# Big-Brother-Pikachu/Where2edit

Hardware: AMD Instinct MI355X
Metric: 1024^2 edited images/sec per mapper step (higher is better)
Workload: dtype f32; 1 GPU; BASELINE configs[1]: FFHQ-1024 StyleGAN2 + clip_loss mapper step (coach.py:79-92), 4 latents/GPU, LevelsMapper, Ranger, id_lambda=0; global_batch=4, per_gpu_batch=4, micro_batch=4, parallelism=dp1, conv_precision=f32, stabilise_steps=12, stabilised=True, hip_graph=True, side_stream=False, clip_precision=f32

## Files before the change

include/w2e.h:

```cpp
#ifndef W2E_H
#define W2E_H

#include <stddef.h>
#include <stdint.h>

#ifdef __cplusplus
extern "C" {
#endif

#define W2E_VERSION 7

int w2e_version(void);
const char* w2e_last_error(void);

int w2e_set_option(const char* name, const char* value);

#define W2E_PLANAR_PITCH(w) ((((w) + 1) + 15) & ~15)
int w2e_get_option(const char* name, int* value);

int w2e_upfirdn2d(const float* x, const float* kern, float* y, int64_t planes, int in_h, int in_w, int out_h,
                  int out_w, int kh, int kw, int up, int down, int pad_x0, int pad_y0, int flip, int in_layout, int in_pitch,
                  int act, const float* out_scale, const float* noise, const float* noise_w, const float* bias,
                  int channels, float slope, float gain, void* stream);
int w2e_blur_adjoint_actbwd(const float* gy, const float* y_fwd, const float* noise, const float* kern, float* gt, float* sums,
                            int64_t planes, int h, int w, float slope, float gain, void* stream);

int w2e_bias_act_fwd(const float* x, const float* bias, const float* noise, const float* noise_w, float* y,
                     int64_t outer, int64_t channels, int64_t inner, float slope, float gain, void* stream);
int w2e_bias_act_bwd(const float* gy, const float* y, float* gx, int64_t n, float slope, float gain, void* stream);
int w2e_bias_act_bwd_reduce(const float* gy, const float* y, const float* noise, float* gx, float* sums,
                            int64_t outer, int64_t channels, int64_t inner, float slope, float gain, void* stream);

int w2e_conv_pack(const float* weight, float* wp, int cout, int cin, float scale, int transpose, int flip,
                  void* stream);

#define W2E_CONV_SAME 0
#define W2E_CONV_UP 1
#define W2E_CONV_DOWN 2

int w2e_modconv3x3(int mode, const float* x, const float* wp, const float* in_scale, const float* out_scale,
                   float* y, int batch, int k_ch, int n_ch, int h, int w, int y_pitch, int act, const float* noise,
                   const float* noise_w, const float* bias, const float* dot_with, float* dot_out, void* stream);

int w2e_wino_weights_fused(const float* wp, float* uf, int k_ch, int n_ch, void* stream);
int w2e_wino_fused(const float* x, const float* in_scale, const float* uf, const float* out_scale, float* y, int batch, int k_ch,
                   int n_ch, int h, int w, int act, const float* noise, const float* noise_w, const float* bias, const float* slope,
                   const float* dot_with, float* dot_out, int wgs, void* stream);

int w2e_wino_gemm_plan(int batch, int k_ch, int n_ch, int h, int w, int* tiles_padded, int* splits, int64_t* workspace_floats);
int w2e_wino_pack_input(const float* x, const float* in_scale, float* vf, int batch, int k_ch, int h, int w, int tiles_padded, void* stream);
int w2e_wino_gemm(const float* uf, const float* vf, const float* out_scale, float* y, int batch, int k_ch, int n_ch, int h, int w,
                  int tiles_padded, int splits, float* workspace, int act, const float* noise, const float* noise_w, const float* bias,
                  const float* slope, const float* dot_with, float* dot_out, void* stream);

int w2e_demod_fwd(const float* s, const float* wsq, float* d, int batch, int cin, int cout, float eps, void* stream);
#define W2E_DEMOD_MAX_LAYERS 32
typedef struct {
    const float* s;
    const float* wsq;
    float* d;
    int cin, cout;
} w2e_demod_layer;
int w2e_demod_all_fwd(const w2e_demod_layer* layers, int n_layers, int batch, float eps, void* stream);
int w2e_demod_bwd(const float* sums, const float* dz, const float* noise_w, const float* bias, const float* d,
                  const float* s, const float* wsq, float* gs, float* gd, int batch, int cin, int cout, void* stream);
// ... 74 lines not shown
```

where2edit_amd/_lib.py:

```python
import ctypes
import os

import torch

from . import build as _build

_P = ctypes.c_void_p
_I = ctypes.c_int
_L = ctypes.c_int64
_F = ctypes.c_float

class DemodLayer(ctypes.Structure):
    _fields_ = [("s", ctypes.c_void_p), ("wsq", ctypes.c_void_p), ("d", ctypes.c_void_p), ("cin", ctypes.c_int), ("cout", ctypes.c_int)]


_PROTOS = {
    "w2e_version": (_I, []),
    "w2e_last_error": (ctypes.c_char_p, []),
    "w2e_set_option": (_I, [ctypes.c_char_p, ctypes.c_char_p]),
    "w2e_get_option": (_I, [ctypes.c_char_p, ctypes.POINTER(ctypes.c_int)]),
    "w2e_upfirdn2d": (_I, [_P, _P, _P, _L, _I, _I, _I, _I, _I, _I, _I, _I, _I, _I, _I, _I, _I, _I, _P, _P, _P, _P, _I, _F, _F, _P]),
    "w2e_blur_adjoint_actbwd": (_I, [_P, _P, _P, _P, _P, _P, _L, _I, _I, _F, _F, _P]),
    "w2e_mapper_pixelnorm": (_I, [_P, _P, _I, _I, _I, _P, _P, _P]),
    "w2e_mapper_linear": (_I, [_I, _P, _P, _P, _P, _P, _I, _I, _I, _P, _P, _F, _F, _I, _P]),
    "w2e_mapper_wgrad": (_I, [_P, _P, _P, _P, _P, _I, _I, _I, _P, _P, _F, _F, _I, _P]),
    "w2e_mapper_gather": (_I, [_P, _P, _I, _I, _I, _P, _P, _P]),
    "w2e_mapper_transpose": (_I, [_P, _I, _P, _P]),
    "w2e_ssmapper_pixelnorm": (_I, [_P, _P, _I, _I, _P, _P]),
    "w2e_ssmapper_gather": (_I, [_P, _P, _I, _I, _P, _P]),
    "w2e_ssmapper_linear": (_I, [_I, _P, _P, _P, _P, _P, _I, _I, _P, _P, _F, _P]),
    "w2e_ssmapper_wgrad": (_I, [_P, _P, _P, _P, _P, _I, _I, _P, _P, _F, _P]),
    "w2e_bias_act_fwd": (_I, [_P, _P, _P, _P, _P, _L, _L, _L, _F, _F, _P]),
    "w2e_bias_act_bwd": (_I, [_P, _P, _P, _L, _F, _F, _P]),
    "w2e_bias_act_bwd_reduce": (_I, [_P, _P, _P, _P, _P, _L, _L, _L, _F, _F, _P]),
    "w2e_conv_pack": (_I, [_P, _P, _I, _I, _F, _I, _I, _P]),
    "w2e_modconv3x3": (_I, [_I, _P, _P, _P, _P, _P, _I, _I, _I, _I, _I, _I, _I, _P, _P, _P, _P, _P, _P]),
    "w2e_wino_weights_fused": (_I, [_P, _P, _I, _I, _P]),
    "w2e_wino_fused": (_I, [_P, _P, _P, _P, _P, _I, _I, _I, _I, _I, _I, _P, _P, _P, _P, _P, _P, _I, _P]),
    "w2e_wino_gemm_plan": (_I, [_I, _I, _I, _I, _I, ctypes.POINTER(ctypes.c_int), ctypes.POINTER(ctypes.c_int), ctypes.POINTER(ctypes.c_int64)]),
    "w2e_wino_pack_input": (_I, [_P, _P, _P, _I, _I, _I, _I, _I, _P]),
    "w2e_wino_gemm": (_I, [_P, _P, _P, _P, _I, _I, _I, _I, _I, _I, _I, _P, _I, _P, _P, _P, _P, _P, _P, _P]),
    "w2e_demod_fwd": (_I, [_P, _P, _P, _I, _I, _I, _F, _P]),
    "w2e_demod_all_fwd": (_I, [ctypes.POINTER(DemodLayer), _I, _I, _F, _P]),
    "w2e_demod_bwd": (_I, [_P, _P, _P, _P, _P, _P, _P, _P, _P, _I, _I, _I, _P]),
    "w2e_modconv_wgrad_plan": (_I, [_I, _I, _I, _I, _I, _I, ctypes.POINTER(ctypes.c_int)]),
    "w2e_modconv_wgrad": (_I, [_I, _P, _P, _P, _P, _P, _I, _I, _I, _I, _I, _I, _P]),
    "w2e_modconv_wgrad_finish": (_I, [_P, _I, _P, _P, _P, _P, _P, _P, _P, _P, _I, _I, _I, _I, _F, _P]),
    "w2e_modconv_wsq": (_I, [_P, _P, _I, _I, _I, _F, _P]),
    "w2e_fromrgb_fwd": (_I, [_P, _P, _P, _P, _I, _I, _L, _F, _P]),
    "w2e_fromrgb_bwd_rows": (_I, [_I, _L]),
    "w2e_fromrgb_bwd": (_I, [_P, _P, _P, _P, _P, _P, _P, _P, _I, _I, _L, _F, _P]),
    "w2e_mbstd_fwd": (_I, [_P, _P, _I, _I, _I, _P]),
    "w2e_mbstd_bwd": (_I, [_P, _P, _P, _I, _I, _I, _P]),
    "w2e_fromrgb_jvp": (_I, [_P, _P, _P, _P, _I, _I, _L, _F, _P]),
    "w2e_mbstd_jvp": (_I, [_P, _P, _P, _I, _I, _I, _P]),
    "w2e_mbstd_hvp": (_I, [_P, _P, _P, _P, _I, _I, _I, _P]),
    "w2e_sumsq_rows_parts": (_I, [_L]),
    "w2e_sumsq_rows": (_I, [_P, _P, _P, _I, _L, _P]),
    "w2e_style_affine_fwd": (_I, [_P, _P, _P, _P, _P, _I, _I, _I, _I, _P]),
# ... 105 lines not shown
```

where2edit_amd/csrc/common.h:

```cpp
#pragma once
#include <hip/hip_runtime.h>
#include <stdarg.h>
#include <stdint.h>
#include <stdio.h>

#include "../../include/w2e.h"

namespace w2e {

void set_error(const char* fmt, ...);

struct Options {
    int conv_precision;
    int deterministic;
    int tune_cfg, tune_cfg_splits, tune_cfg_mode;
    int tune_upall, tune_dma, tune_fuse;
    int tune_mw;
    int tune_xcd;
    int tune_print, tune_blur, tune_gemm_s;
    int tune_skip, tune_clock;
};
const Options& options();

static inline bool big_lds_once(const void* fn, unsigned* done_mask) {
    int dev = 0;
    if (hipGetDevice(&dev) != hipSuccess || dev < 0 || dev >= 32) return false;
    if (*done_mask & (1u << dev)) return true;
    if (hipFuncSetAttribute(fn, hipFuncAttributeMaxDynamicSharedMemorySize, 160 * 1024) != hipSuccess) return false;
    *done_mask |= 1u << dev;
    return true;
}

int cu_count();

#define W2E_REQUIRE(cond, ...)        \
    do {                              \
        if (!(cond)) {                \
            w2e::set_error(__VA_ARGS__); \
            return 1;                 \
// ... 25 lines not shown
```

where2edit_amd/csrc/modconv.hip:

```cpp
#include <math.h>
#include <stdlib.h>
#include <string.h>

#include <type_traits>

#include "common.h"
#include "../../include/w2e_irse.h"

namespace w2e {

typedef float f32x16 __attribute__((ext_vector_type(16)));

struct ConvParams {
    const float* x;
    const float* wp;
    const float* in_scale;
    const float* out_scale;
    float* y;
    const float* noise;
    const float* noise_w;
    const float* bias;
    const float* dot_with;
    float* dot_out;
    int batch, K, N;
    int H, W;
    int in_h, in_w;
    int out_h, out_w;
    int th, tw, tw_log2;
    int tiles_x, tiles_y, tiles_n;
    int ph, pw, plane;
    unsigned pw_magic;
    int border_wgs, groups_row, groups_col;
    int tune_skip;
    const float* slope;
    int in_off;
    int splits, k_per;
    unsigned long long* stamps;
};

enum { EPI_PLAIN = 0, EPI_ACT = 1, EPI_DOT = 2, EPI_PRELU = 3 };

constexpr int CONV_UPALL = 3;
#ifdef W2E_TUNING
#define W2E_SKIP(p, bit) ((p).tune_skip & (bit))
#else
#define W2E_SKIP(p, bit) false
#endif
#ifdef W2E_STAMPS
constexpr int STAMP_STRIDE = 8;
#else
constexpr int STAMP_STRIDE = 4;
#endif
__host__ __device__ constexpr bool is_up(int mode) { return mode == W2E_CONV_UP || mode == CONV_UPALL; }

__host__ __device__ constexpr int max_patch_slots(int mode, int tm, int nt) {
    return mode == W2E_CONV_DOWN ? (nt == 512 ? (tm >= 1024 ? 9 : 5) : (tm >= 512 ? 9 : (tm >= 256 ? 5 : (tm >= 128 ? 3 : (tm >= 64 ? 2 : 1)))))
                                 : (nt == 512 ? (tm >= 2048 ? 5 : (tm >= 1024 ? 3 : 2)) : (tm >= 512 ? 3 : (tm >= 256 ? 2 : 1)));
}

template <int MODE, int PY, int PX>
// ... 221 lines not shown
    const bool even_ok = is_row ? v <= p.W : v < p.H, odd_ok = is_row ? v < p.W : v < p.H;
    const int e_idx = is_row ? (0 * hp + p.H) * wpp + v : (0 * hp + v) * wpp + p.W;
    const int o_idx = is_row ? (1 * hp + p.H) * wpp + v : (2 * hp + v) * wpp + p.W;
    constexpr int RPW = 32 / NW;
#pragma unroll
    for (int q = 0; q < RPW; ++q) {
        const int rr = wave * RPW + q;
        const int r = rr & 15;
        float sum = 0.f;
#pragma unroll
        for (int w = 0; w < NW; ++w) sum += red[w][rr][lane];
        const int och = ob * 32 + (r & 3) + 8 * (r >> 2) + 4 * half;
        if (och >= p.N) continue;
        const float os = p.out_scale ? p.out_scale[(int64_t)b * p.N + och] : 1.f;
        float* yp = p.y + ((int64_t)b * p.N + och) * 4 * hp * wpp;
        if (rr < 16) {
            if (even_ok) yp[e_idx] = sum * os;
        } else if (odd_ok) {
            yp[o_idx] = sum * os;
        }
    }
}

template <int MODE, int EPI, int NOB, int NPB, int WO, int WP, int KC, int DMA>
__global__ __launch_bounds__(64 * WO * WP, 2) void modconv_kernel(ConvParams p) {
    constexpr int NT = 64 * WO * WP;
    constexpr int TN = 32 * NOB * WO;
    constexpr int NPX = (MODE == CONV_UPALL) ? NPB / 4 : NPB;
    constexpr int MAXX = max_patch_slots(MODE == CONV_UPALL ? W2E_CONV_UP : MODE, 32 * NPX * WP, NT);
    extern __shared__ __attribute__((aligned(16))) float smem[];
    constexpr int WS_FLOATS = (MODE == W2E_CONV_UP ? 32 : KC * 9) * TN;
    float4* ws = reinterpret_cast<float4*>(smem);
    float4* xs = reinterpret_cast<float4*>(smem + WS_FLOATS);

    const int tid = threadIdx.x, lane = tid & 63;
    const int wave = __builtin_amdgcn_readfirstlane(tid >> 6);
    const int half = lane >> 5, j = lane & 31;
    const int wo = wave / WP, wpx = wave % WP;

    int bid = blockIdx.x;
    if (is_up(MODE)) {
        if (bid < p.border_wgs) {
            if (W2E_SKIP(p, 32)) return;
            upconv_border<NT>(p, smem, bid);
            return;
        }
        bid -= p.border_wgs;
    }
    const int per_phase = (gridDim.x - p.border_wgs) >> 2;
    const int phase = (MODE == W2E_CONV_UP) ? bid / per_phase : 0;
    if (MODE == W2E_CONV_UP) bid -= phase * per_phase;
    const int ks = bid % p.splits;
    bid /= p.splits;
    const int k_lo = ks * p.k_per;
    const int k_hi = W2E_SKIP(p, 2) ? k_lo : ((k_lo + p.k_per < p.K) ? k_lo + p.k_per : p.K);
#ifdef W2E_TUNING
    if (p.stamps && tid == 0) {
        p.stamps[STAMP_STRIDE * (int64_t)blockIdx.x + 0] = __builtin_amdgcn_s_memtime();
        p.stamps[STAMP_STRIDE * (int64_t)blockIdx.x + 1] = __builtin_amdgcn_s_memrealtime();
    }
#endif
    const int tx = bid % p.tiles_x;
    bid /= p.tiles_x;
    const int ty = bid % p.tiles_y;
    bid /= p.tiles_y;
    const int b = bid % p.batch;
    const int nt = bid / p.batch;
    const int n0 = nt * TN;
    const int r0 = ty * p.th, c0 = tx * p.tw;

    int base[NPB];
#pragma unroll
    for (int pb = 0; pb < NPX; ++pb) {
        const int m = (wpx * NPX + pb) * 32 + j;
        const int ly = m >> p.tw_log2, lx = m & (p.tw - 1);
        const bool ok = ly < p.th && r0 + ly < p.H && c0 + lx < p.W;
        int off;
        if (MODE == W2E_CONV_SAME) off = ly * p.pw + lx;
        else if (is_up(MODE)) off = (ly + 1) * p.pw + lx + 1;
        else off = 2 * ly * p.pw + 2 * lx;
        if (!ok) off = is_up(MODE) ? p.pw + 1 : 0;
        base[pb] = half * p.plane + off;
    }

    f32x16 acc[NOB][NPB];
#pragma unroll
    for (int ob = 0; ob < NOB; ++ob)
#pragma unroll
        for (int pb = 0; pb < NPB; ++pb)
#pragma unroll
            for (int r = 0; r < 16; ++r) acc[ob][pb][r] = 0.f;

    const int64_t in_plane = (int64_t)p.in_h * p.in_w;
    const int patch = p.ph * p.pw;
    const int oy0 = (MODE == W2E_CONV_DOWN) ? 2 * r0 + p.in_off : r0 - 1;
    const int ox0 = (MODE == W2E_CONV_DOWN) ? 2 * c0 + p.in_off : c0 - 1;

    auto k_loop = [&](auto py_c, auto px_c) __attribute__((always_inline)) {
        constexpr int PY = decltype(py_c)::value, PX = decltype(px_c)::value;
// ... 310 lines not shown
            p.stamps[STAMP_STRIDE * (int64_t)blockIdx.x + 4] = st_wait;
            p.stamps[STAMP_STRIDE * (int64_t)blockIdx.x + 5] = st_bar;
            p.stamps[STAMP_STRIDE * (int64_t)blockIdx.x + 6] = __builtin_amdgcn_s_memtime() - st_t0;
            p.stamps[STAMP_STRIDE * (int64_t)blockIdx.x + 7] = st_issue;
        }
#endif
    };
    using I0 = std::integral_constant<int, 0>;
    using I1 = std::integral_constant<int, 1>;
    if constexpr (DMA) {
        static_assert(MODE != W2E_CONV_UP, "the per-phase UP form keeps the register pipeline");
        dma_loop(0);
    } else if (MODE == W2E_CONV_UP) {
        switch (phase) {
            case 0: k_loop(I0{}, I0{}); break;
            case 1: k_loop(I0{}, I1{}); break;
            case 2: k_loop(I1{}, I0{}); break;
            default: k_loop(I1{}, I1{}); break;
        }
    } else {
        k_loop(I0{}, I0{});
    }

    const float nw = (EPI == EPI_ACT && p.noise) ? p.noise_w[0] * 1.4142135623730951f : 0.f;
    float* red = smem;
    if (EPI == EPI_DOT) {
        __syncthreads();
        if (tid < TN) red[tid] = 0.f;
        __syncthreads();
    }
    int gy[NPB], gx[NPB];
    bool valid[NPB];
#pragma unroll
    for (int pb = 0; pb < NPB; ++pb) {
        const int m = (wpx * NPX + pb % NPX) * 32 + j;
        const int ly = m >> p.tw_log2, lx = m & (p.tw - 1);
        gy[pb] = r0 + ly;
        gx[pb] = c0 + lx;
        valid[pb] = ly < p.th && gy[pb] < p.H && gx[pb] < p.W;
    }
    int pix[NPB];
    float nz[NPB];
#pragma unroll
    for (int pb = 0; pb < NPB; ++pb) {
        const int ph_pb = (MODE == CONV_UPALL) ? pb / NPX : phase;
        if (is_up(MODE)) pix[pb] = (ph_pb * (p.H + 1) + gy[pb]) * W2E_PLANAR_PITCH(p.W) + gx[pb];
// ... 109 lines not shown
                                 int transpose, int flip) {
    const int Kd = transpose ? cout : cin, Nd = transpose ? cin : cout;
    const int64_t total = (int64_t)((Kd + 7) / 8) * 9 * 2 * Nd * 4;
    for (int64_t e = (int64_t)blockIdx.x * blockDim.x + threadIdx.x; e < total; e += (int64_t)gridDim.x * blockDim.x) {
        const int c = (int)(e & 3);
        const int n = (int)((e >> 2) % Nd);
        const int hh = (int)((e / (4 * (int64_t)Nd)) & 1);
        const int tap = (int)((e / (8 * (int64_t)Nd)) % 9);
        const int kc = (int)(e / (72 * (int64_t)Nd));
        const int k = kc * 8 + 2 * c + hh;
        float v = 0.f;
        if (k < Kd) {
            const int o = transpose ? k : n, i = transpose ? n : k;
            v = scale * w[((int64_t)o * cin + i) * 9 + (flip ? 8 - tap : tap)];
        }
        wp[e] = v;
    }
}

struct TileCfg {
    int nob, npb, wo, wp;
};

template <int MODE, int EPI, int NOB, int NPB, int WO, int WP, int KC, int DMA = 0>
static void launch_cfg(const ConvParams& p, int grid, size_t lds, hipStream_t s) {
    if (lds > 64 * 1024) {
        static unsigned done = 0;
        big_lds_once((const void*)modconv_kernel<MODE, EPI, NOB, NPB, WO, WP, KC, DMA>, &done);
    }
    modconv_kernel<MODE, EPI, NOB, NPB, WO, WP, KC, DMA><<<grid, 64 * WO * WP, lds, s>>>(p);
}

static bool dma_has_cfg(bool all_phase, int cfg) {
    return all_phase ? (cfg == 0 || cfg == 1 || cfg == 2 || cfg == 8 || cfg == 11)
                     : (cfg == 0 || cfg == 1 || cfg == 2 || cfg == 8 || cfg == 9 || cfg == 10);
}

template <int EPI>
static bool launch_x3_down(int cfg, const ConvParams& p, int grid, size_t lds, hipStream_t s) {
    if (cfg != 9) return false;
    launch_cfg<W2E_CONV_DOWN, EPI, 2, 2, 2, 4, 8, 2>(p, grid, lds, s);
    return true;
}

static bool launch_x3_up(int cfg, const ConvParams& p, int grid, size_t lds, hipStream_t s) {
    switch (cfg) {
        case 0: launch_cfg<CONV_UPALL, EPI_PLAIN, 2, 4, 2, 4, 8, 2>(p, grid, lds, s); return true;
        case 1: launch_cfg<CONV_UPALL, EPI_PLAIN, 2, 4, 1, 8, 8, 2>(p, grid, lds, s); return true;
        case 2: launch_cfg<CONV_UPALL, EPI_PLAIN, 1, 4, 1, 8, 8, 2>(p, grid, lds, s); return true;
        case 11: launch_cfg<CONV_UPALL, EPI_PLAIN, 1, 8, 1, 8, 8, 2>(p, grid, lds, s); return true;
    }
    return false;
}
// ... 397 lines not shown
#define W2E_CHECK_UP_PITCH(name)                                                                                                       \
    W2E_REQUIRE(mode != W2E_CONV_UP || y_pitch == W2E_PLANAR_PITCH(w),                                                                 \
                name ": UP output with a row pitch of %d floats, this library's layout has %d (W2E_PLANAR_PITCH, ABI %d): rebuild the caller", \
                y_pitch, W2E_PLANAR_PITCH(w), W2E_VERSION)

extern "C" int w2e_modconv3x3(int mode, const float* x, const float* wp, const float* in_scale, const float* out_scale,
                              float* y, int batch, int k_ch, int n_ch, int h, int w, int y_pitch, int act, const float* noise,
                              const float* noise_w, const float* bias, const float* dot_with, float* dot_out,
                              void* stream) {
    W2E_CHECK_UP_PITCH("modconv3x3");
    return conv_impl(mode, x, wp, in_scale, out_scale, y, batch, k_ch, n_ch, h, w, act, noise, noise_w, bias, dot_with, dot_out,
                     nullptr, 0, 0, stream);
}

extern "C" int w2e_conv3x3(int mode, const float* x, const float* wp, const float* in_scale, const float* out_scale, float* y,
                           int batch, int k_ch, int n_ch, int h, int w, int y_pitch, int down_pad, const float* bias, const float* slope,
                           void* stream) {
    W2E_CHECK_UP_PITCH("conv3x3");
    const int prelu = (bias || slope) ? 1 : 0;
    W2E_REQUIRE(!(prelu && mode == W2E_CONV_UP), "conv3x3: no bias / PReLU epilogue in UP mode");
    return conv_impl(mode, x, wp, in_scale, out_scale, y, batch, k_ch, n_ch, h, w, 0, nullptr, nullptr, bias, nullptr, nullptr,
                     slope, prelu, down_pad, stream);
}
```

where2edit_amd/csrc/runtime.hip:

```cpp
#include <stdlib.h>
#include <string.h>

#include "common.h"

namespace w2e {

static thread_local char g_err[512] = "";

void set_error(const char* fmt, ...) {
    va_list ap;
    va_start(ap, fmt);
    vsnprintf(g_err, sizeof(g_err), fmt, ap);
    va_end(ap);
}

static Options g_opt;

static int parse_precision(const char* v) { return (v && strcmp(v, "bf16x3") == 0) ? 1 : 0; }

static bool apply(Options& o, const char* name, const char* value) {
    const int iv = value ? atoi(value) : 0;
    if (!strcmp(name, "conv_precision")) o.conv_precision = parse_precision(value);
    else if (!strcmp(name, "deterministic")) o.deterministic = iv != 0;
    else if (!strcmp(name, "tune_cfg")) {
        o.tune_cfg = -1, o.tune_cfg_splits = 1, o.tune_cfg_mode = -1;
        if (value && *value) sscanf(value, "%d,%d,%d", &o.tune_cfg, &o.tune_cfg_splits, &o.tune_cfg_mode);
    } else if (!strcmp(name, "tune_upall")) o.tune_upall = (value && *value) ? iv : -1;
    else if (!strcmp(name, "tune_dma")) o.tune_dma = (value && *value) ? iv : -1;
    else if (!strcmp(name, "tune_print")) o.tune_print = iv;
    else if (!strcmp(name, "tune_blur")) o.tune_blur = iv;
    else if (!strcmp(name, "tune_gemm_s")) o.tune_gemm_s = iv;
    else if (!strcmp(name, "tune_fuse")) o.tune_fuse = (value && *value) ? iv : -1;
    else if (!strcmp(name, "tune_xcd")) o.tune_xcd = (value && *value) ? iv : -1;
    else if (!strcmp(name, "tune_mw")) o.tune_mw = (value && *value) ? iv : -1;
#ifdef W2E_TUNING
    else if (!strcmp(name, "tune_skip")) o.tune_skip = iv;
    else if (!strcmp(name, "tune_clock")) o.tune_clock = iv;
#endif
    else return false;
    return true;
}

static Options from_env() {
    Options o{};
    o.tune_cfg = -1, o.tune_cfg_splits = 1, o.tune_cfg_mode = -1, o.tune_upall = -1, o.tune_dma = -1, o.tune_fuse = -1, o.tune_xcd = -1, o.tune_mw = -1;
    static const char* const kEnv[][2] = {
        {"W2E_CONV_PRECISION", "conv_precision"}, {"W2E_DETERMINISTIC", "deterministic"}, {"W2E_TUNE_CFG", "tune_cfg"},
        {"W2E_TUNE_UPALL", "tune_upall"},         {"W2E_TUNE_DMA", "tune_dma"},           {"W2E_TUNE_PRINT", "tune_print"},
        {"W2E_TUNE_BLUR", "tune_blur"},           {"W2E_TUNE_GEMM_S", "tune_gemm_s"},     {"W2E_TUNE_FUSE", "tune_fuse"},
        {"W2E_TUNE_SKIP", "tune_skip"},           {"W2E_TUNE_CLOCK", "tune_clock"},       {"W2E_TUNE_XCD", "tune_xcd"},
        {"W2E_TUNE_MW", "tune_mw"}};
    for (const auto& e : kEnv)
        if (const char* v = getenv(e[0])) apply(o, e[1], v);
    return o;
}

struct OptionsInit {
    OptionsInit() { g_opt = from_env(); }
};
static OptionsInit g_opt_init;

const Options& options() { return g_opt; }

int cu_count() {
    static int cached[32];
    int dev = 0;
    if (hipGetDevice(&dev) != hipSuccess || dev < 0 || dev >= 32) return 256;
    if (!cached[dev]) {
        hipDeviceProp_t prop;
        cached[dev] = (hipGetDeviceProperties(&prop, dev) == hipSuccess && prop.multiProcessorCount > 0) ? prop.multiProcessorCount : 256;
    }
    return cached[dev];
}

// ... 21 lines not shown
}

}

extern "C" {

int w2e_version(void) { return W2E_VERSION; }
const char* w2e_last_error(void) { return w2e::g_err; }

int w2e_set_option(const char* name, const char* value) {
    W2E_REQUIRE(name != nullptr, "set_option: null name");
    W2E_REQUIRE(w2e::apply(w2e::g_opt, name, value), "set_option: unknown option '%s'", name);
    return 0;
}

int w2e_get_option(const char* name, int* value) {
    W2E_REQUIRE(name && value, "get_option: null argument");
    const w2e::Options& o = w2e::g_opt;
    if (!strcmp(name, "conv_precision")) *value = o.conv_precision;
    else if (!strcmp(name, "deterministic")) *value = o.deterministic;
    else if (!strcmp(name, "tune_cfg")) *value = o.tune_cfg;
    else if (!strcmp(name, "tune_fuse")) *value = o.tune_fuse;
    else if (!strcmp(name, "tune_blur")) *value = o.tune_blur;
    else if (!strcmp(name, "tuning_build")) {
#ifdef W2E_TUNING
        *value = 1;
#else
        *value = 0;
#endif
    } else W2E_REQUIRE(false, "get_option: unknown option '%s'", name);
    return 0;
}

}
```

where2edit_amd/functional.py:

```python
import ctypes
import math
import os

import torch
from torch.autograd.function import once_differentiable

from . import _lib, profiling
from ._lib import call, ptr, stream_ptr

SQRT2 = math.sqrt(2.0)

_NOGRAD_PREFIX = 0
_POISON = os.environ.get("W2E_DEBUG_POISON", "0") == "1"


def set_debug_poison(on=True):
    global _POISON
    _POISON = bool(on)


def _grad_rows(shape, n_skip, device, like=None):
    buf = torch.empty(shape, device=device, dtype=torch.float32) if like is None else torch.empty_like(like)
    if _POISON and n_skip:
        buf[:n_skip].fill_(float("nan"))
# ... 311 lines not shown
        y = torch.empty((b, n, 2, 2, h + 1, planar_pitch(w)), device=x.device, dtype=torch.float32)
    elif out is not None:
        y = out
    else:
        y = torch.empty((b, n, h, w), device=x.device, dtype=torch.float32)
    dot = None
    if dot_with is not None:
        dot = dot_out if dot_out is not None else torch.zeros((b, n), device=x.device, dtype=torch.float32)
    noise = noise_w = bias = None
    if act is not None:
        noise, noise_w, bias = act
    form = _wino_form(x, k, n, h, w, dot_with) if mode == MODE_SAME else 0
    sp = profiling.span("modconv3x3_wino4" if form else "modconv3x3", 2.0 * b * k * n * 9 * h * w)
    if form:
        _modconv_wino(form, x, wp, in_scale, out_scale, y, k, n, h, w, act, dot_with, dot)
    else:
        call("w2e_modconv3x3", mode, ptr(x), ptr(wp), ptr(in_scale), ptr(out_scale), ptr(y), b, k, n, h, w,
             y.shape[-1] if mode == MODE_UP else 0, int(act is not None), ptr(noise), ptr(noise_w), ptr(bias), ptr(dot_with), ptr(dot), stream_ptr())
    if sp is not None:
        sp.end()
    return y, dot


def _channel_dot(a, b, out=None):
    n, c = a.shape[0], a.shape[1]
    if out is None:
        out = torch.empty((n, c), device=a.device, dtype=torch.float32)
    call("w2e_channel_sums", ptr(a), ptr(b), ptr(out), n, c, a.shape[2] * a.shape[3], stream_ptr())
    return out


def _scale_planes(a, s):
    n, c = a.shape[0], a.shape[1]
    out = torch.empty_like(a)
    zero = torch.zeros((n, c), device=a.device, dtype=torch.float32)
    call("w2e_se_apply_bwd", ptr(a), ptr(_c(s)), ptr(zero), ptr(out), n, c, a.shape[2] * a.shape[3], stream_ptr())
    return out


def demod_coefficients(s, wsq, eps=1e-8):
    b, cin = s.shape
    cout = wsq.shape[0]
    d = torch.empty((b, cout), device=s.device, dtype=torch.float32)
    call("w2e_demod_fwd", ptr(s), ptr(wsq), ptr(d), b, cin, cout, float(eps), stream_ptr())
    return d

# ... 69 lines not shown
        self.gpre = self.sums = None
        if gpre is None:
            return None
        if gpre is not gout:
            raise RuntimeError("where2edit_amd: the gradient of a StyledConv output that was routed through its ToRGB node "
                               "(ActLink) reached the StyledConv backward as a different tensor -- a tensor hook, retain_grad() "
                               "or a second consumer on that activation is not supported on the fused training path "
                               "(use return_features=True / the unfused modules to tap activations)")
        return sums


class _StyledConv(torch.autograd.Function):

    @staticmethod
    def forward(ctx, x, s, wsq, noise, noise_w, bias, packs, blur_kernel, upsample, fuse_act, link=None, d_pre=None, weight=None,
                wscale=1.0):
        x, s = _c(x), _c(s)
        b, cin, h, w = x.shape
        wp_f, wp_b = packs
        d = None
        if wsq is not None:
            d = d_pre if d_pre is not None else demod_coefficients(s, wsq)
        act = (noise, noise_w, bias) if fuse_act else None
        if upsample:
            t, _ = _modconv_raw(MODE_UP, x, wp_f, s, d, h, w)
            if w >= 16:
                out = _upfirdn2d_raw(t, blur_kernel, 2 * h, 2 * w, 1, 1, 1, 1, True,
                                     act=((None,) + act) if fuse_act else None, planar_hw=(2 * h + 1, 2 * w + 1))
            else:
                out = _upfirdn2d_raw(unplanar(t, w), blur_kernel, 2 * h, 2 * w, 1, 1, 1, 1, True,
                                     act=((None,) + act) if fuse_act else None)
        else:
            out, _ = _modconv_raw(MODE_SAME, x, wp_f, s, d, h, w, act=act)
        ctx.save_for_backward(x, s, d, wsq, noise, noise_w, bias, out, wp_b, blur_kernel, weight)
        ctx.cfg = (upsample, fuse_act)
        ctx.wscale = float(wscale)
        ctx.link = link
        ctx.n_skip = _NOGRAD_PREFIX if _NOGRAD_PREFIX < b else 0
        ctx.pool = _GRAD_POOL
        return out

    @staticmethod
    @once_differentiable
    def backward(ctx, gout):
        x, s, d, wsq, noise, noise_w, bias, out, wp_b, blur_kernel, weight = ctx.saved_tensors
        upsample, fuse_act = ctx.cfg
        n_skip, full = ctx.n_skip, x.shape[0]
# ... 267 lines not shown
```

where2edit_amd/profiling.py:

```python
import os
import sys
import tempfile

import torch

_active = None


class KernelTimer:

    def __init__(self):
        self.records = []
        self.enabled = True

    def __enter__(self):
        global _active
        _active = self
        return self

    def __exit__(self, *exc):
        global _active
        _active = None

    def summary(self):
# ... 3 lines not shown
            calls, ms, tot = out.get(name, (0, 0.0, 0.0))
            out[name] = (calls + 1, ms + a.elapsed_time(b), tot + work)
        return out


class _Span:
    __slots__ = ("name", "work", "start")

    def __init__(self, name, work):
        self.name, self.work = name, work
        self.start = torch.cuda.Event(enable_timing=True)
        self.start.record()

    def end(self):
        e = torch.cuda.Event(enable_timing=True)
        e.record()
        _active.records.append((self.name, self.work, self.start, e))


def span(name, work=0.0):
    return _Span(name, work) if (_active is not None and _active.enabled) else None


SELECTION_PREFIXES = ("modconv mode", "modconv variant", "wino_fused variant", "upfirdn variant", "  ")


def conv_selections(fn):
    from . import _lib
    from . import functional as K
    torch.cuda.synchronize()
    sys.stderr.flush()
    with tempfile.TemporaryFile(mode="w+b") as tmp:
        saved = os.dup(2)
        os.dup2(tmp.fileno(), 2)
        try:
            _lib.set_option("tune_print", 1)
            K.WINO_LOG = []
            fn()
            torch.cuda.synchronize()
        finally:
            _lib.set_option("tune_print", 0)
            wino, K.WINO_LOG = K.WINO_LOG, None
            os.dup2(saved, 2)
            os.close(saved)
        tmp.seek(0)
        lines = [ln for ln in tmp.read().decode().splitlines() if ln.startswith(SELECTION_PREFIXES)]
    return lines, wino
# ... 1 lines not shown
```

Baseline: 260.7 images/s.

## Fuse upsampling modconv with 4x4 blur and bias/noise/lrelu epilogue

Adds a fused kernel variant in which the transposed (upsampling) modulated conv writes its output tile to LDS and then applies the 4x4 FIR blur plus noise, bias and leaky-ReLU epilogue before storing. Overlapping tiles (halo of one input pixel per side) avoid a second launch and the round trip of the large intermediate through global memory. It is enabled automatically for the highest-resolution layers (K<=64, N<=32, >=512x512 input). The cost is recomputation on tile halos, heavy LDS use that may lower occupancy, and a runtime separability check on the kernel.

```diff
diff --git a/include/w2e.h b/include/w2e.h
--- a/include/w2e.h
+++ b/include/w2e.h
@@ -41,6 +41,11 @@
 int w2e_modconv3x3(int mode, const float* x, const float* wp, const float* in_scale, const float* out_scale,
                    float* y, int batch, int k_ch, int n_ch, int h, int w, int y_pitch, int act, const float* noise,
                    const float* noise_w, const float* bias, const float* dot_with, float* dot_out, void* stream);
+
+int w2e_modconv_upblur_plan(int batch, int k_ch, int n_ch, int h, int w, int* fused);
+int w2e_modconv_upblur(const float* x, const float* wp, const float* in_scale, const float* out_scale, const float* kern,
+                       float* y, int batch, int k_ch, int n_ch, int h, int w, const float* noise, const float* noise_w,
+                       const float* bias, void* stream);
 
 int w2e_wino_weights_fused(const float* wp, float* uf, int k_ch, int n_ch, void* stream);
 int w2e_wino_fused(const float* x, const float* in_scale, const float* uf, const float* out_scale, float* y, int batch, int k_ch,
diff --git a/where2edit_amd/_lib.py b/where2edit_amd/_lib.py
--- a/where2edit_amd/_lib.py
+++ b/where2edit_amd/_lib.py
@@ -35,6 +35,8 @@
     "w2e_bias_act_bwd_reduce": (_I, [_P, _P, _P, _P, _P, _L, _L, _L, _F, _F, _P]),
     "w2e_conv_pack": (_I, [_P, _P, _I, _I, _F, _I, _I, _P]),
     "w2e_modconv3x3": (_I, [_I, _P, _P, _P, _P, _P, _I, _I, _I, _I, _I, _I, _I, _P, _P, _P, _P, _P, _P]),
+    "w2e_modconv_upblur_plan": (_I, [_I, _I, _I, _I, _I, ctypes.POINTER(ctypes.c_int)]),
+    "w2e_modconv_upblur": (_I, [_P, _P, _P, _P, _P, _P, _I, _I, _I, _I, _I, _P, _P, _P, _P]),
     "w2e_wino_weights_fused": (_I, [_P, _P, _I, _I, _P]),
     "w2e_wino_fused": (_I, [_P, _P, _P, _P, _P, _I, _I, _I, _I, _I, _I, _P, _P, _P, _P, _P, _P, _I, _P]),
     "w2e_wino_gemm_plan": (_I, [_I, _I, _I, _I, _I, ctypes.POINTER(ctypes.c_int), ctypes.POINTER(ctypes.c_int), ctypes.POINTER(ctypes.c_int64)]),
diff --git a/where2edit_amd/csrc/common.h b/where2edit_amd/csrc/common.h
--- a/where2edit_amd/csrc/common.h
+++ b/where2edit_amd/csrc/common.h
@@ -15,6 +15,7 @@
     int deterministic;
     int tune_cfg, tune_cfg_splits, tune_cfg_mode;
     int tune_upall, tune_dma, tune_fuse;
+    int tune_upblur;
     int tune_mw;
     int tune_xcd;
     int tune_print, tune_blur, tune_gemm_s;
diff --git a/where2edit_amd/csrc/modconv.hip b/where2edit_amd/csrc/modconv.hip
--- a/where2edit_amd/csrc/modconv.hip
+++ b/where2edit_amd/csrc/modconv.hip
@@ -36,6 +36,8 @@
     int in_off;
     int splits, k_per;
     unsigned long long* stamps;
+    const float* fir;
+    int vec4;
 };
 
 enum { EPI_PLAIN = 0, EPI_ACT = 1, EPI_DOT = 2, EPI_PRELU = 3 };
@@ -303,7 +305,7 @@
     }
 }
 
-template <int MODE, int EPI, int NOB, int NPB, int WO, int WP, int KC, int DMA>
+template <int MODE, int EPI, int NOB, int NPB, int WO, int WP, int KC, int DMA, int UPB = 0>
 __global__ __launch_bounds__(64 * WO * WP, 2) void modconv_kernel(ConvParams p) {
     constexpr int NT = 64 * WO * WP;
     constexpr int TN = 32 * NOB * WO;
@@ -320,7 +322,7 @@
     const int wo = wave / WP, wpx = wave % WP;
 
     int bid = blockIdx.x;
-    if (is_up(MODE)) {
+    if (is_up(MODE) && !UPB) {
         if (bid < p.border_wgs) {
             if (W2E_SKIP(p, 32)) return;
             upconv_border<NT>(p, smem, bid);
@@ -348,14 +350,14 @@
     const int b = bid % p.batch;
     const int nt = bid / p.batch;
     const int n0 = nt * TN;
-    const int r0 = ty * p.th, c0 = tx * p.tw;
+    const int r0 = UPB ? ty * (p.th - 2) - 1 : ty * p.th, c0 = UPB ? tx * (p.tw - 2) - 1 : tx * p.tw;
 
     int base[NPB];
 #pragma unroll
     for (int pb = 0; pb < NPX; ++pb) {
         const int m = (wpx * NPX + pb) * 32 + j;
         const int ly = m >> p.tw_log2, lx = m & (p.tw - 1);
-        const bool ok = ly < p.th && r0 + ly < p.H && c0 + lx < p.W;
+        const bool ok = UPB || (ly < p.th && r0 + ly < p.H && c0 + lx < p.W);
         int off;
         if (MODE == W2E_CONV_SAME) off = ly * p.pw + lx;
         else if (is_up(MODE)) off = (ly + 1) * p.pw + lx + 1;
@@ -712,6 +714,154 @@
         k_loop(I0{}, I0{});
     }
 
+    if constexpr (UPB) {
+        static_assert(MODE == CONV_UPALL && EPI == EPI_PLAIN && NOB == 1 && NPB == 8 && WO == 1 && WP == 8 && DMA == 1, "the blur epilogue is written for tile {1,8,1,8}");
+        typedef float f32x2 __attribute__((ext_vector_type(2)));
+        typedef float f32x4 __attribute__((ext_vector_type(4)));
+        typedef int i32x4 __attribute__((ext_vector_type(4)));
+        constexpr int TPITCH = 64, CHS = 32 * TPITCH;
+        constexpr int GCH = 16, SROWS = 14, NSTRIP = 2, QUADS = 15, ITEMS = NSTRIP * GCH * QUADS;
+        constexpr unsigned OOB = 0x80000000u;
+        constexpr float kGainF = 1.4142135623730951f, kSlope = 0.2f;
+        const int out_w = 2 * p.W, out_h = 2 * p.H;
+        const unsigned oplane = (unsigned)out_h * (unsigned)out_w;
+        const bool vec = p.vec4 != 0;
+        const bool worker = tid < ITEMS;
+        const int strip = tid / (GCH * QUADS), rem = tid - strip * (GCH * QUADS);
+        const int ch = rem / QUADS, qi = rem - ch * QUADS;
+        const int Y0 = 2 * (r0 + 1) + strip * SROWS, X0 = 2 * (c0 + 1) + 4 * qi;
+        float kr[16], kh[4], kv[4];
+#pragma unroll
+        for (int i = 0; i < 16; ++i) kr[i] = p.fir[15 - i];
+        bool separable = kr[0] != 0.f;
+        {
+            float kmax = 0.f;
+#pragma unroll
+            for (int i = 0; i < 16; ++i) kmax = fmaxf(kmax, fabsf(kr[i]));
+#pragma unroll
+            for (int i = 0; i < 4; ++i) kh[i] = kr[i], kv[i] = separable ? kr[4 * i] / kr[0] : 0.f;
+#pragma unroll
+            for (int i = 0; i < 16; ++i) separable = separable && fabsf(kr[i] - kv[i >> 2] * kh[i & 3]) <= 1e-7f * kmax;
+        }
+        float* const nzs = smem + GCH * CHS;
+        float* const oss = nzs + NSTRIP * SROWS * QUADS * 4;
+        const bool has_os = p.out_scale != nullptr;
+        const __amdgpu_buffer_rsrc_t rbs = __builtin_amdgcn_make_buffer_rsrc(const_cast<float*>(p.bias ? p.bias : p.x), (short)0, p.bias ? p.N * 4 : 0, 0x00020000);
+        float eb2[2];
+#pragma unroll
+        for (int g = 0; g < 2; ++g) eb2[g] = __builtin_bit_cast(float, __builtin_amdgcn_raw_buffer_load_b32(rbs, (unsigned)(n0 + GCH * g + ch) * 4u, 0, 0)) * kGainF;
+        const float nw = p.noise ? p.noise_w[0] * kGainF : 0.f;
+        const __amdgpu_buffer_rsrc_t rn = __builtin_amdgcn_make_buffer_rsrc(const_cast<float*>(p.noise ? p.noise : p.x), (short)0, p.noise ? (int)(oplane * 4u) : 0, 0x00020000);
+        float nzv[4] = {0.f, 0.f, 0.f, 0.f};
+        float osv = 1.f;
+        {
+            const int nq = tid / QUADS, ni = tid - nq * QUADS;
+            const int ny = 2 * (r0 + 1) + nq, nx = 2 * (c0 + 1) + 4 * ni;
+            const unsigned no = (nq < NSTRIP * SROWS && ny < out_h && nx < out_w) ? ((unsigned)ny * (unsigned)out_w + (unsigned)nx) * 4u : OOB;
+            if (vec) {
+                const f32x4 n4 = __builtin_bit_cast(f32x4, __builtin_amdgcn_raw_buffer_load_b128(rn, no, 0, 0));
+                nzv[0] = n4[0], nzv[1] = n4[1], nzv[2] = n4[2], nzv[3] = n4[3];
+            } else {
+#pragma unroll
+                for (int e = 0; e < 4; ++e)
+                    nzv[e] = __builtin_bit_cast(float, __builtin_amdgcn_raw_buffer_load_b32(rn, (no != OOB && nx + e < out_w) ? no + 4u * e : OOB, 0, 0));
+            }
+            if (has_os && tid < 32) osv = n0 + tid < p.N ? p.out_scale[(int64_t)b * p.N + n0 + tid] : 0.f;
+        }
+        const bool col_ok = worker && X0 < out_w;
+        const unsigned p0 = ((unsigned)Y0 * (unsigned)out_w + (unsigned)X0) * 4u;
+        const __amdgpu_buffer_rsrc_t ry = __builtin_amdgcn_make_buffer_rsrc(p.y + (int64_t)b * p.N * oplane, (short)0, (int)((unsigned)p.N * oplane * 4u), 0x00020000);
+        __syncthreads();
+        if (tid < NSTRIP * SROWS * QUADS) *reinterpret_cast<f32x4*>(nzs + 4 * tid) = f32x4{nzv[0], nzv[1], nzv[2], nzv[3]};
+        if (tid < 32) oss[tid] = osv;
+        auto put = [&](auto gc) __attribute__((always_inline)) {
+            constexpr int G = decltype(gc)::value;
+#pragma unroll
+            for (int rr = 0; rr < 8; ++rr) {
+                const int r = 8 * G + rr;
+                const int c = (rr & 3) + 8 * (rr >> 2) + 4 * half;
+                const float osr = oss[GCH * G + c];
+                float* tc = smem + c * CHS + 2 * j;
+#pragma unroll
+                for (int pb = 0; pb < 2; ++pb)
+#pragma unroll
+                    for (int py = 0; py < 2; ++py) {
+                        const int row = 2 * (wave * 2 + pb) + py;
+                        f32x2 v;
+                        v[0] = acc[0][(2 * py + 0) * 2 + pb][r] * osr;
+                        v[1] = acc[0][(2 * py + 1) * 2 + pb][r] * osr;
+                        *reinterpret_cast<f32x2*>(tc + row * TPITCH) = v;
+                    }
+            }
+        };
+        auto fir = [&](auto sep_c, int g, float eb) __attribute__((always_inline)) {
+            constexpr bool SEP = decltype(sep_c)::value;
+            const bool ch_ok = n0 + GCH * g + ch < p.N;
+            const unsigned choff = (unsigned)(n0 + GCH * g + ch) * oplane * 4u;
+            const float* tb = smem + ch * CHS + (strip * SROWS + 1) * TPITCH + 4 * qi;
+            f32x4 o[4];
+#pragma unroll
+            for (int s = 0; s < 4; ++s) o[s] = f32x4{0.f, 0.f, 0.f, 0.f};
+#pragma unroll
+            for (int k = 0; k < SROWS + 3; ++k) {
+                const f32x4 wa = *reinterpret_cast<const f32x4*>(tb + k * TPITCH), wb = *reinterpret_cast<const f32x4*>(tb + k * TPITCH + 4);
+                const float w[8] = {wa[0], wa[1], wa[2], wa[3], wb[0], wb[1], wb[2], wb[3]};
+                if (SEP) {
+                    f32x4 h;
+#pragma unroll
+                    for (int e = 0; e < 4; ++e) h[e] = kh[0] * w[e + 1] + kh[1] * w[e + 2] + kh[2] * w[e + 3] + kh[3] * w[e + 4];
+#pragma unroll
+                    for (int a = 0; a < 4; ++a)
+                        if (k - a >= 0 && k - a < SROWS) o[(k - a) & 3] += kv[a] * h;
+                } else {
+#pragma unroll
+                    for (int a = 0; a < 4; ++a)
+                        if (k - a >= 0 && k - a < SROWS) {
+#pragma unroll
+                            for (int e = 0; e < 4; ++e)
+                                o[(k - a) & 3][e] += kr[4 * a] * w[e + 1] + kr[4 * a + 1] * w[e + 2] + kr[4 * a + 2] * w[e + 3] + kr[4 * a + 3] * w[e + 4];
+                        }
+                }
+                if (k >= 3) {
+                    const int q = k - 3;
+                    const f32x4 acc4 = o[q & 3];
+                    o[q & 3] = f32x4{0.f, 0.f, 0.f, 0.f};
+                    const f32x4 nz = *reinterpret_cast<const f32x4*>(nzs + ((strip * SROWS + q) * QUADS + qi) * 4);
+                    float v[4];
+#pragma unroll
+                    for (int e = 0; e < 4; ++e) {
+                        const float t = acc4[e] * kGainF + eb + nw * nz[e];
+                        v[e] = fmaxf(t, t * kSlope);
+                    }
+                    const unsigned vo = (ch_ok && col_ok && Y0 + q < out_h) ? p0 + choff + (unsigned)(q * out_w) * 4u : OOB;
+                    if (vec) {
+                        f32x4 v4;
+                        v4[0] = v[0], v4[1] = v[1], v4[2] = v[2], v4[3] = v[3];
+                        __builtin_amdgcn_raw_buffer_store_b128(__builtin_bit_cast(i32x4, v4), ry, vo, 0, 0);
+                    } else {
+#pragma unroll
+                        for (int e = 0; e < 4; ++e)
+                            __builtin_amdgcn_raw_buffer_store_b32(__builtin_bit_cast(int, v[e]), ry, (vo != OOB && X0 + e < out_w) ? vo + 4u * e : OOB, 0, 0);
+                    }
+                }
+            }
+        };
+        using B0 = std::integral_constant<bool, false>;
+        using B1 = std::integral_constant<bool, true>;
+#pragma unroll
+        for (int g = 0; g < 2; ++g) {
+            __syncthreads();
+            if (g == 0) put(std::integral_constant<int, 0>{});
+            else put(std::integral_constant<int, 1>{});
+            __syncthreads();
+            if (worker) {
+                if (separable) fir(B1{}, g, eb2[g]);
+                else fir(B0{}, g, eb2[g]);
+            }
+        }
+        return;
+    }
+
     const float nw = (EPI == EPI_ACT && p.noise) ? p.noise_w[0] * 1.4142135623730951f : 0.f;
     float* red = smem;
     if (EPI == EPI_DOT) {
@@ -867,13 +1017,13 @@
     int nob, npb, wo, wp;
 };
 
-template <int MODE, int EPI, int NOB, int NPB, int WO, int WP, int KC, int DMA = 0>
+template <int MODE, int EPI, int NOB, int NPB, int WO, int WP, int KC, int DMA = 0, int UPB = 0>
 static void launch_cfg(const ConvParams& p, int grid, size_t lds, hipStream_t s) {
     if (lds > 64 * 1024) {
         static unsigned done = 0;
-        big_lds_once((const void*)modconv_kernel<MODE, EPI, NOB, NPB, WO, WP, KC, DMA>, &done);
-    }
-    modconv_kernel<MODE, EPI, NOB, NPB, WO, WP, KC, DMA><<<grid, 64 * WO * WP, lds, s>>>(p);
+        big_lds_once((const void*)modconv_kernel<MODE, EPI, NOB, NPB, WO, WP, KC, DMA, UPB>, &done);
+    }
+    modconv_kernel<MODE, EPI, NOB, NPB, WO, WP, KC, DMA, UPB><<<grid, 64 * WO * WP, lds, s>>>(p);
 }
 
 static bool dma_has_cfg(bool all_phase, int cfg) {
@@ -1317,3 +1467,67 @@
     return conv_impl(mode, x, wp, in_scale, out_scale, y, batch, k_ch, n_ch, h, w, 0, nullptr, nullptr, bias, nullptr, nullptr,
                      slope, prelu, down_pad, stream);
 }
+
+namespace w2e {
+constexpr int UPB_TH = 16, UPB_TW = 32;
+
+static const char* upblur_refusal(const Options& opt, int batch, int k_ch, int n_ch, int h, int w) {
+    if (batch < 0 || k_ch <= 0 || n_ch <= 0 || h <= 0 || w <= 0) return "bad dims";
+    if (opt.conv_precision != 0) return "conv_precision = bf16x3 keeps the two-launch form";
+    if (opt.tune_cfg >= 0 && opt.tune_cfg_splits > 1 && (opt.tune_cfg_mode < 0 || opt.tune_cfg_mode == W2E_CONV_UP)) return "split-K keeps the two-launch form";
+    if (((int64_t)k_ch + 8) * h * w * 4 >= ((int64_t)1 << 32)) return "one image of the input exceeds 4 GB";
+    if ((int64_t)n_ch * 4 * h * w * 4 >= ((int64_t)1 << 31)) return "one image of the output exceeds 2 GB";
+    if ((int64_t)batch * ceil_div(n_ch, 32) * ceil_div(h, UPB_TH - 2) * ceil_div(w, UPB_TW - 2) >= ((int64_t)1 << 31)) return "too many tiles";
+    return nullptr;
+}
+
+static bool upblur_auto(const Options& opt, int k_ch, int n_ch, int h, int w) {
+    if (opt.tune_cfg >= 0 || opt.tune_upall == 0 || opt.tune_dma == 0) return false;
+    return k_ch <= 64 && n_ch <= 32 && (int64_t)h * w >= 512 * 512;
+}
+}
+
+extern "C" int w2e_modconv_upblur_plan(int batch, int k_ch, int n_ch, int h, int w, int* fused) {
+    W2E_REQUIRE(fused != nullptr, "modconv_upblur_plan: null argument");
+    const Options& opt = options();
+    *fused = 0;
+    if (opt.tune_upblur == 0 || upblur_refusal(opt, batch, k_ch, n_ch, h, w)) return 0;
+    *fused = (opt.tune_upblur > 0 || upblur_auto(opt, k_ch, n_ch, h, w)) ? 1 : 0;
+    return 0;
+}
+
+extern "C" int w2e_modconv_upblur(const float* x, const float* wp, const float* in_scale, const float* out_scale, const float* kern,
+                                  float* y, int batch, int k_ch, int n_ch, int h, int w, const float* noise, const float* noise_w,
+                                  const float* bias, void* stream) {
+    W2E_REQUIRE(x && wp && kern && y, "modconv_upblur: null tensor");
+    W2E_REQUIRE(!noise || noise_w, "modconv_upblur: noise without noise_w");
+    const Options& opt = options();
+    const char* why = upblur_refusal(opt, batch, k_ch, n_ch, h, w);
+    W2E_REQUIRE(!why, "modconv_upblur: %s (K %d N %d %dx%d B %d)", why, k_ch, n_ch, h, w, batch);
+    if (batch == 0) return 0;
+    ConvParams p{};
+    p.x = x, p.wp = wp, p.in_scale = in_scale, p.out_scale = out_scale, p.y = y;
+    p.noise = noise, p.noise_w = noise_w, p.bias = bias, p.fir = kern;
+    p.batch = batch, p.K = k_ch, p.N = n_ch, p.H = h, p.W = w;
+    p.in_h = h, p.in_w = w, p.out_h = 2 * h, p.out_w = 2 * w;
+    p.th = UPB_TH, p.tw = UPB_TW, p.tw_log2 = 5;
+    p.tiles_x = (int)ceil_div(w, UPB_TW - 2), p.tiles_y = (int)ceil_div(h, UPB_TH - 2), p.tiles_n = (int)ceil_div(n_ch, 32);
+    p.ph = UPB_TH + 1, p.pw = UPB_TW + 1;
+    p.plane = (p.ph * p.pw + 15) & ~15;
+    p.pw_magic = (unsigned)(((uint64_t)1 << 32) / (unsigned)p.pw + 1);
+    p.splits = 1, p.k_per = (int)(ceil_div(k_ch, 8) * 8);
+    p.vec4 = ((2 * w) % 4 == 0 && ((uintptr_t)y & 15) == 0 && ((uintptr_t)noise & 15) == 0) ? 1 : 0;
+    size_t lds = sizeof(float) * (2 * ((size_t)8 * 9 * 32 + (size_t)8 * p.plane) + (size_t)((k_ch + 7) / 8) * 8);
+    const int groups = 2;
+    const size_t lds_epi = sizeof(float) * (16 * 32 * 64 + 28 * 60 + 32);
+    if (lds < lds_epi) lds = lds_epi;
+    W2E_REQUIRE(lds <= 160 * 1024, "modconv_upblur: K = %d needs %zu B of LDS", k_ch, lds);
+    const int64_t grid = (int64_t)p.tiles_x * p.tiles_y * p.tiles_n * batch;
+    if (opt.tune_print) {
+        fprintf(stderr, "modconv mode %d (all-phase) K %d N %d %dx%d B %d -> cfg 11 splits 1\n", W2E_CONV_UP, k_ch, n_ch, h, w, batch);
+        fprintf(stderr, "modconv upblur variant cfg 11 th %d tw %d groups %d vec %d K %d N %d %dx%d B %d\n", p.th, p.tw, groups, p.vec4, k_ch, n_ch, h, w, batch);
+    }
+    launch_cfg<CONV_UPALL, EPI_PLAIN, 1, 8, 1, 8, 8, 1, 1>(p, (int)grid, lds, (hipStream_t)stream);
+    W2E_LAUNCH_CHECK("modconv_upblur");
+    return 0;
+}
diff --git a/where2edit_amd/csrc/runtime.hip b/where2edit_amd/csrc/runtime.hip
--- a/where2edit_amd/csrc/runtime.hip
+++ b/where2edit_amd/csrc/runtime.hip
@@ -33,6 +33,7 @@
     else if (!strcmp(name, "tune_fuse")) o.tune_fuse = (value && *value) ? iv : -1;
     else if (!strcmp(name, "tune_xcd")) o.tune_xcd = (value && *value) ? iv : -1;
     else if (!strcmp(name, "tune_mw")) o.tune_mw = (value && *value) ? iv : -1;
+    else if (!strcmp(name, "tune_upblur")) o.tune_upblur = (value && *value) ? iv : -1;
 #ifdef W2E_TUNING
     else if (!strcmp(name, "tune_skip")) o.tune_skip = iv;
     else if (!strcmp(name, "tune_clock")) o.tune_clock = iv;
@@ -43,13 +44,13 @@
 
 static Options from_env() {
     Options o{};
-    o.tune_cfg = -1, o.tune_cfg_splits = 1, o.tune_cfg_mode = -1, o.tune_upall = -1, o.tune_dma = -1, o.tune_fuse = -1, o.tune_xcd = -1, o.tune_mw = -1;
+    o.tune_cfg = -1, o.tune_cfg_splits = 1, o.tune_cfg_mode = -1, o.tune_upall = -1, o.tune_dma = -1, o.tune_fuse = -1, o.tune_xcd = -1, o.tune_mw = -1, o.tune_upblur = -1;
     static const char* const kEnv[][2] = {
         {"W2E_CONV_PRECISION", "conv_precision"}, {"W2E_DETERMINISTIC", "deterministic"}, {"W2E_TUNE_CFG", "tune_cfg"},
         {"W2E_TUNE_UPALL", "tune_upall"},         {"W2E_TUNE_DMA", "tune_dma"},           {"W2E_TUNE_PRINT", "tune_print"},
         {"W2E_TUNE_BLUR", "tune_blur"},           {"W2E_TUNE_GEMM_S", "tune_gemm_s"},     {"W2E_TUNE_FUSE", "tune_fuse"},
         {"W2E_TUNE_SKIP", "tune_skip"},           {"W2E_TUNE_CLOCK", "tune_clock"},       {"W2E_TUNE_XCD", "tune_xcd"},
-        {"W2E_TUNE_MW", "tune_mw"}};
+        {"W2E_TUNE_MW", "tune_mw"},               {"W2E_TUNE_UPBLUR", "tune_upblur"}};
     for (const auto& e : kEnv)
         if (const char* v = getenv(e[0])) apply(o, e[1], v);
     return o;
@@ -117,6 +118,7 @@
     else if (!strcmp(name, "tune_cfg")) *value = o.tune_cfg;
     else if (!strcmp(name, "tune_fuse")) *value = o.tune_fuse;
     else if (!strcmp(name, "tune_blur")) *value = o.tune_blur;
+    else if (!strcmp(name, "tune_upblur")) *value = o.tune_upblur;
     else if (!strcmp(name, "tuning_build")) {
 #ifdef W2E_TUNING
         *value = 1;
diff --git a/where2edit_amd/functional.py b/where2edit_amd/functional.py
--- a/where2edit_amd/functional.py
+++ b/where2edit_amd/functional.py
@@ -357,6 +357,27 @@
     return y, dot
 
 
+def _upblur_planned(b, k, n, h, w):
+    fused = ctypes.c_int(0)
+    call("w2e_modconv_upblur_plan", b, k, n, h, w, ctypes.byref(fused))
+    return bool(fused.value)
+
+
+def _modconv_upblur_raw(x, wp, in_scale, out_scale, kernel, h, w, act):
+    b, k = x.shape[0], x.shape[1]
+    n = wp.shape[3]
+    if wp.shape[0] != (k + 7) // 8:
+        raise RuntimeError(f"modconv: packed weight holds {wp.shape[0]} 8-channel groups, input has {k} channels")
+    noise, noise_w, bias = act
+    y = torch.empty((b, n, 2 * h, 2 * w), device=x.device, dtype=torch.float32)
+    sp = profiling.span("modconv3x3", 2.0 * b * k * n * 9 * h * w)
+    call("w2e_modconv_upblur", ptr(x), ptr(wp), ptr(in_scale), ptr(out_scale), ptr(kernel), ptr(y), b, k, n, h, w,
+         ptr(noise), ptr(noise_w), ptr(bias), stream_ptr())
+    if sp is not None:
+        sp.end()
+    return y
+
+
 def _channel_dot(a, b, out=None):
     n, c = a.shape[0], a.shape[1]
     if out is None:
@@ -472,7 +493,9 @@
         if wsq is not None:
             d = d_pre if d_pre is not None else demod_coefficients(s, wsq)
         act = (noise, noise_w, bias) if fuse_act else None
-        if upsample:
+        if upsample and fuse_act and tuple(blur_kernel.shape) == (4, 4) and _upblur_planned(b, cin, wp_f.shape[3], h, w):
+            out = _modconv_upblur_raw(x, wp_f, s, d, blur_kernel, h, w, act)
+        elif upsample:
             t, _ = _modconv_raw(MODE_UP, x, wp_f, s, d, h, w)
             if w >= 16:
                 out = _upfirdn2d_raw(t, blur_kernel, 2 * h, 2 * w, 1, 1, 1, 1, True,
diff --git a/where2edit_amd/profiling.py b/where2edit_amd/profiling.py
--- a/where2edit_amd/profiling.py
+++ b/where2edit_amd/profiling.py
@@ -49,7 +49,7 @@
     return _Span(name, work) if (_active is not None and _active.enabled) else None
 
 
-SELECTION_PREFIXES = ("modconv mode", "modconv variant", "wino_fused variant", "upfirdn variant", "  ")
+SELECTION_PREFIXES = ("modconv mode", "modconv variant", "modconv upblur variant", "wino_fused variant", "upfirdn variant", "  ")
 
 
 def conv_selections(fn):
```

Result: faster. 263.4 images/s, median of 6 (+1.0%).
